# RajaeeKh/TriNerfLet

Measured on AMD Instinct MI355X. Metric: train rays/sec (whole node), higher is better.
Workload: dtype f16; 1 GPU; base: 3x32ch x 2048^2 planes, bior6.8 scale 32, hidden 64, 60000 rays/step/GPU, solid-sphere occupancy r=0.8 (re-imposed after each refresh), fp16 planes + fp16 MFMA MLP, fp32 masters, Adam+L1; GT colours = an analytic function of the ray direction (synthetic.target_colors), not a second seeded field's render; sample_budget_M=4769546, parallelism=ray-dp1

## Files before the change

include/trinerflet_hip.h:

```cpp
#ifndef TRINERFLET_HIP_H
#define TRINERFLET_HIP_H

#include <stdint.h>

#ifdef __cplusplus
extern "C" {
#endif

#define TNL_API __attribute__((visibility("default")))

TNL_API int tnl_abi_version(void);


TNL_API int tnl_near_far_from_aabb(const float *rays_o, const float *rays_d, const float *aabb,
                                   uint32_t N, float min_near, float *nears, float *fars,
                                   void *stream);

TNL_API int tnl_sph_from_ray(const float *rays_o, const float *rays_d, float radius, uint32_t N,
                             float *coords, void *stream);

TNL_API int tnl_morton3D(const int32_t *coords, uint32_t N, int32_t *indices, void *stream);

TNL_API int tnl_morton3D_invert(const int32_t *indices, uint32_t N, int32_t *coords, void *stream);

// ... 180 lines not shown
                              const float *abs_sum, float l1_coef, float *reg, void *stream);

TNL_API uint64_t tnl_permute_index(uint64_t g, uint64_t total, uint64_t key);
TNL_API int tnl_ray_batch(const float *poses, const float *intrinsics_host, uint32_t B, uint32_t H, uint32_t W,
                          const void *images, int channels, int images_u8, const int64_t *pix, uint64_t first,
                          uint64_t perm_total, uint64_t perm_key, uint32_t N, float bg_color,
                          const float *bg_rand, float *rays_o, float *rays_d, float *gt_rgb, int64_t *pix_out,
                          void *stream);

TNL_API int tnl_render_work(int units);

TNL_API int tnl_render_rays(const void *planes_tm, int half_in, uint32_t C, uint32_t R, uint32_t Hd, uint32_t Hc,
                            const void *packed, const float *rays_o, const float *rays_d, const float *nears,
                            const float *fars, uint32_t N, const uint8_t *grid, float bound, float dt_gamma,
                            uint32_t max_steps, uint32_t cascades, uint32_t H, float T_thresh, float density_scale,
                            const float *noises, int32_t *queue, float *weights_sum, float *depth, float *image,
                            void *stream);

TNL_API int tnl_infer_plan(int32_t *state, uint32_t N, uint32_t max_steps, uint32_t min_step, void *stream);
TNL_API int tnl_march_rays_dev(const int32_t *state, uint32_t N, const int32_t *rays_alive, const float *rays_t,
                               const float *rays_o, const float *rays_d, float bound, float dt_gamma,
                               uint32_t max_steps, uint32_t C, uint32_t H, const uint8_t *grid, const float *fars,
                               float *xyzs, float *dirs, float *deltas, const float *noises, float *t_scratch,
                               uint32_t rows_cap, void *stream);
TNL_API int tnl_composite_rays_dev(const int32_t *state, uint32_t N, float T_thresh, int32_t *rays_alive,
                                   float *rays_t, const float *sigmas, const float *rgbs, const float *deltas,
                                   float *weights_sum, float *depth, float *image, void *stream);
TNL_API int tnl_compact_rays_dev(int32_t *state, uint32_t N, const int32_t *rays_alive, int32_t *rays_alive_out,
                                 int32_t *workspace, void *stream);

TNL_API int tnl_idwt_level_forward_win(const float *x, const float *yh, uint32_t S, uint32_t n, int wave, float *out,
                                       const int32_t *win, void *stream);
TNL_API int tnl_idwt_level_backward_win(const float *dout, uint32_t S, uint32_t n, int wave, float *dx, float *dyh,
                                        const int32_t *win, int strided, int32_t *out_rect, void *stream);

TNL_API int tnl_idwt_set_walk_min_n(uint32_t walk_min_n);
TNL_API int tnl_idwt_get_walk_min_n(void);
TNL_API int tnl_idwt_level_forward_spans(const float *x, const float *yh, uint32_t S, uint32_t n, int wave, void *out,
                                         int half_out, const int32_t *win, int strided, const int32_t *spans,
                                         void *stream);
TNL_API int tnl_idwt_level_backward_spans(const float *dout, uint32_t S, uint32_t n, int wave, float *dx, float *dyh,
                                          const int32_t *win, int strided, int32_t *out_rect, const int32_t *spans,
                                          void *stream);
TNL_API int tnl_idwt_level_backward_live_adam(const float *dout, uint32_t S, uint32_t n, int wave, float *dx,
                                              const int32_t *win, int strided, const int32_t *live_rect,
                                              const int32_t *spans, float *p, float *m, float *v,
                                              const int32_t *band_table, uint32_t nb, const float *step_rec,
                                              float beta1, float beta2, float eps, float inv_scale,
                                              const float *inv_scale_dev, float l1_coef, const float *found_inf,
                                              float *abs_sum, void *stream);
TNL_API int tnl_planes_half_to_texel_major_spans(const void *planes_roi_half, uint32_t C, uint32_t R,
                                                 void *planes_tm_half, const int32_t *roi, const int32_t *spans,
                                                 void *stream);
TNL_API int tnl_idwt_set_tuning(int key, int value);
TNL_API int tnl_adam_l1_step_rect(float *p, float *grad, float *m, float *v, uint32_t S, uint32_t bands, uint32_t n,
                                  uint32_t spp, uint32_t s0, const int32_t *rect, float lr,
                                  const float *opt_step_dev, float beta1, float beta2, float eps, float inv_scale,
                                  const float *inv_scale_dev, float l1_coef, const float *found_inf,
                                  float *abs_sum, void *stream);
TNL_API int tnl_adam_record_step_dev(float *ring, int32_t slot, const float *lr_dev, const float *opt_step_dev, float beta1,
                                     float beta2, const float *found_inf, void *stream);
TNL_API int tnl_adam_l1_step_rec(float *p, float *grad, float *m, float *v, uint64_t n, const float *step_rec, float beta1,
                                 float beta2, float eps, const float *inv_scale_dev, float l1_coef,
                                 const float *found_inf, float *abs_sum, void *stream);
TNL_API int tnl_adam_l1_step_rect_rec(float *p, float *grad, float *m, float *v, uint32_t S, uint32_t bands, uint32_t n,
                                      uint32_t spp, uint32_t s0, const int32_t *rect, const float *step_rec, float beta1,
                                      float beta2, float eps, const float *inv_scale_dev, float l1_coef,
                                      const float *found_inf, float *abs_sum, void *stream);
TNL_API int tnl_adam_l1_step_live(float *p, float *grad, float *m, float *v, uint32_t S, uint32_t spp, uint32_t s0,
                                  uint32_t n_levels, const uint64_t *offsets, const uint32_t *sizes,
                                  const uint32_t *bands, const int32_t *live, const int32_t *grad_rect,
                                  const float *l1_coefs, float lr, const float *opt_step_dev, const float *step_rec,
                                  float beta1, float beta2, float eps, float inv_scale, const float *inv_scale_dev,
                                  const float *found_inf, float *abs_sum, void *stream);
TNL_API int tnl_adam_record_step(float *ring, int32_t slot, float lr, const float *opt_step_dev, float beta1,
                                 float beta2, const float *found_inf, void *stream);
TNL_API int tnl_adam_record_step_l1(float *ring, int32_t slot, float lr, const float *opt_step_dev, float beta1,
                                    float beta2, const float *found_inf, const float *l1_scaled_dev,
                                    const float *inv_scale_dev, void *stream);
TNL_API int tnl_adam_l1_catchup(float *p, float *m, float *v, uint32_t S, uint32_t bands, uint32_t n, uint32_t spp,
                                uint32_t s0, const int32_t *live, const float *ring, int32_t count, float beta1,
                                float beta2, float eps, float l1_coef, float *abs_sums, void *stream);
TNL_API int tnl_adam_l1_step_live_bands(float *p, float *grad, float *m, float *v, uint32_t S, uint32_t spp, uint32_t s0,
                                        uint32_t n_levels, const uint64_t *offsets, const uint32_t *sizes,
                                        const uint32_t *bands, const int32_t *live, const int32_t *grad_rect,
                                        const int32_t *const *band_tables, const uint32_t *band_quads,
                                        const float *l1_coefs, float lr, const float *opt_step_dev, const float *step_rec,
                                        float beta1, float beta2, float eps, float inv_scale, const float *inv_scale_dev,
                                        const float *found_inf, float *abs_sum, void *stream);
TNL_API int tnl_adam_l1_catchup_bands(float *p, float *m, float *v, uint32_t S, uint32_t bands, uint32_t n, uint32_t spp,
                                      uint32_t s0, const int32_t *live, const int32_t *band_table, const float *ring,
                                      int32_t count, float beta1, float beta2, float eps, float l1_coef, float *abs_sums,
                                      void *stream);

#ifdef __cplusplus
}
#endif
#endif
```

trinerflet_amd/_step/common.py:

```python
import ctypes as C_
import math
import types

import numpy as np

import torch
import torch.distributed as dist

from .. import _lib as L
from .. import distributed as D
from .. import occupancy
from .. import raymarching
from ..nerf import field as F_
from ..triplaneencoder.triplane_encoder import (_IDWTLevel, _ToTexelMajor, half_roi_into_texel_major, half_to_texel_major,
                                                idwt_level_half, idwt_level_half_roi)


def lr_factor(it, iters, warmup_steps, sched_base=0.1, warmup_factor=1e-3, sched_exp=2.5):
    w = max(warmup_steps, 0)
    if it < w:
        return sched_base * warmup_factor + it * (1 - warmup_factor) / (w - 1)
    return sched_base ** (min((it - w) / iters, 1) ** sched_exp)


class _Flat:

    def __init__(self, params):
        self.params = list(params)
        dev = self.params[0].device
        sizes = [p.numel() for p in self.params]
        self.offsets, off = [], 0
        for n in sizes:
            self.offsets.append(off)
            off += (n + 3) // 4 * 4
        self.total = off
        self.data = torch.zeros(off, dtype=torch.float32, device=dev)
        self.grad = torch.zeros(off, dtype=torch.float32, device=dev)
        self.m = torch.zeros(off, dtype=torch.float32, device=dev)
        self.v = torch.zeros(off, dtype=torch.float32, device=dev)
        for p, o, n in zip(self.params, self.offsets, sizes):
            self.data[o:o + n].copy_(p.data.reshape(-1))
            p.data = self.data[o:o + n].view(p.shape)
        self.sizes = sizes

    def grad_view(self, k):
        o, n = self.offsets[k], self.sizes[k]
        return self.grad[o:o + n].view(self.params[k].shape)

    def tune_placement(self, time_pass, candidates=12, spacing=3, good_gbs=5900.0):
        nbytes = 28.0 * self.total
        gbs = lambda ms: nbytes / (ms * 1e-3) / 1e9
        t0 = time_pass(self.data, self.grad, self.m, self.v)
        report = {"before_ms": round(t0, 4), "before_GBs": round(gbs(t0), 1), "tried_ms": []}
        best_t, best = t0, None
        hold = []
        if gbs(t0) < good_gbs:
            need = (spacing + 2) * self.data.numel() * 4
            for _ in range(candidates):
                if torch.cuda.mem_get_info(self.data.device)[0] < need:
                    report["stopped"] = "free memory"
                    break
                cand = torch.empty_like(self.data)
                hold.append(cand)
                hold.extend(torch.empty_like(self.data) for _ in range(spacing))
                t = time_pass(cand, self.grad, self.m, self.v)
                report["tried_ms"].append(round(t, 4))
                if t < best_t:
                    best_t, best = t, cand
# ... 44 lines not shown
```

trinerflet_amd/_step/planes.py:

```python
from .common import (C_, D, F_, L, _Flat, _IDWTLevel, _StepState, _ToTexelMajor, dist, half_roi_into_texel_major,
                     half_to_texel_major, idwt_level_half, idwt_level_half_roi, lr_factor, math, np, occupancy, raymarching,
                     torch, types)


class PlanesMixin:

    def _idwt_level_win(self, x, yh, win, s0=0, spans=None):
        x = x.detach().contiguous()
        yh = yh.detach().contiguous()
        P, Cc, n = x.shape[0], x.shape[1], x.shape[-1]
        out = torch.empty(P, Cc, 2 * n, 2 * n, dtype=torch.float32, device=x.device)
        L.check(L.lib().tnl_idwt_level_forward_spans(L.ptr(x), L.ptr(yh), L.u32(P * Cc), L.u32(n),
                                                     L.i32(self.enc.wave_id), L.ptr(out), L.i32(0),
                                                     L.roi_array(list(win) + [self.C, s0]), L.i32(1), L.ptr(spans),
                                                     L.stream()),
                "idwt_level_forward_spans")
        return out

    def _cropped(self, lvl):
        return self.base_res > 0 and self.crop_k > 0 and self.coef.params[lvl].shape[-1] < self.base_res

    def _crop(self, x, lvl):
        if not self._cropped(lvl):
            return x
        k = self.crop_k
        return x[..., k:-k, k:-k].contiguous()

    def rebuild_planes(self, roi=False):
        enc = self.enc
        fast = (self.J > 0 and enc.plane_dtype == torch.float16 and self.C % 8 == 0 and self.R % 16 == 0)
        if self._roi_request is not None:
            self._roi = self._finish_roi()
        roi = roi and self._roi is not None and self._tm_full is not None
        if not roi:
            self.flush_deferred()
        with torch.no_grad():
            wins = self._forward_windows() if roi else [None] * self.J
            spans, plane_spans = self._forward_spans() if roi else ([None] * self.J, None)
            if self.dist_mode == "sharded":
                planes = self._rebuild_sharded(roi, wins, spans)
            else:
                x = enc.planes_features
                for lvl in range(self.J):
                    yh = enc.planes_features_wavelet_coefs[lvl]
                    if fast and lvl == self.J - 1:
                        x = idwt_level_half_roi(x, yh, enc.wave_id, self._roi10(), spans[lvl]) if roi else \
                            idwt_level_half(x, yh, enc.wave_id)
                    elif wins[lvl] is not None:
                        x = self._idwt_level_win(x, yh, wins[lvl], spans=spans[lvl])
                    else:
                        x = _IDWTLevel.apply(x, yh, enc.wave_id)
                    x = self._crop(x, lvl)
                planes = x
            if roi:
                enc.last_used_planes = None
                enc._planes_tm = None
                enc._planes_tm_window = None
                if planes.dtype == torch.float16:
                    return half_roi_into_texel_major(planes, self._tm_full, self._roi10(), plane_spans)
                L.check(L.lib().tnl_planes_to_texel_major_win(L.ptr(planes), L.u32(self.C), L.u32(self.R), L.i32(0),
                                                              L.ptr(self._tm_full), L.roi_array(self._roi10()), L.stream()),
                        "planes_to_texel_major_win")
                return self._tm_full
            if planes.dtype == torch.float16:
                enc.last_used_planes = None
                enc._planes_tm = half_to_texel_major(planes)
            else:
                enc.last_used_planes = planes
                enc._planes_tm = _ToTexelMajor.apply(planes, enc.plane_dtype == torch.float16)
            enc._planes_tm_window = None
            self._tm_full = enc._planes_tm if self.use_roi else None
        return enc._planes_tm

    def _slice_range(self):
        return D.slice_range(3 * self.C, self.world, self.rank)

    def _rebuild_sharded(self, roi=False, wins=None, spans=None):
        enc = self.enc
        spans = spans if spans is not None else [None] * self.J
        s0, s1 = self._slice_range()
        n0 = enc.planes_features.shape[-1]
        x = enc.planes_features.reshape(3 * self.C, n0, n0)[s0:s1].unsqueeze(0).contiguous()
        fast = (self.J > 0 and enc.plane_dtype == torch.float16 and self.C % 8 == 0 and self.R % 16 == 0)
        for lvl in range(self.J):
            n = x.shape[-1]
            yh = enc.planes_features_wavelet_coefs[lvl].reshape(3 * self.C, 3, n, n)[s0:s1].unsqueeze(0).contiguous()
            if fast and lvl == self.J - 1:
                x = idwt_level_half_roi(x, yh, enc.wave_id, self._roi10(s0), spans[lvl]) if roi else \
                    idwt_level_half(x, yh, enc.wave_id)
            elif wins is not None and wins[lvl] is not None:
                x = self._idwt_level_win(x, yh, wins[lvl], s0, spans[lvl])
            else:
                x = _IDWTLevel.apply(x, yh, enc.wave_id)
            x = self._crop(x, lvl)
        if roi and x.dtype == torch.float16:
            return D.all_gather_slices(x.reshape(s1 - s0, self._roi[7], self._roi[6]), self.pg)
        if roi:
            r, C = self._roi, self.C
            xs = x.reshape(s1 - s0, self.R, self.R)
            mine = torch.empty(s1 - s0, r[7], r[6], dtype=torch.float32, device=x.device)
            for pl in range(3):
                a0, a1 = max(pl * C, s0), min((pl + 1) * C, s1)
                if a1 > a0:
                    mine[a0 - s0:a1 - s0] = xs[a0 - s0:a1 - s0, r[3 + pl]:r[3 + pl] + r[7], r[pl]:r[pl] + r[6]]
            allw = D.all_gather_slices(mine, self.pg)
            full = torch.empty(3, C, self.R, self.R, dtype=torch.float32, device=x.device)
            for pl in range(3):
                full[pl, :, r[3 + pl]:r[3 + pl] + r[7], r[pl]:r[pl] + r[6]] = allw[pl * C:(pl + 1) * C]
            return full
        mine = x.reshape(s1 - s0, self.R, self.R)
        return D.all_gather_slices(mine, self.pg).view(3, self.C, self.R, self.R)

    def _adjoint(self, grad_tm, g_cm=None, fuse=None, roi=None, scattered=False, live_adam=None):
        lib = L.lib()
        C, R = self.C, self.R
        if g_cm is None:
            g_cm = torch.empty(3, C, R, R, dtype=torch.float32, device=self.dev)
# ... 120 lines not shown
```

trinerflet_amd/csrc/wavelet.hip:

```cpp
#include <hip/hip_fp16.h>
#include <hip/hip_runtime.h>
#include <stdint.h>
#ifndef TNL_MAIN_PRIO
#define TNL_MAIN_PRIO 0
#endif
#ifndef TNL_PRIO_FWD
#define TNL_PRIO_FWD TNL_MAIN_PRIO
#endif
#ifndef TNL_PRIO_BWD
#define TNL_PRIO_BWD TNL_MAIN_PRIO
#endif
#define TNL_SET_PRIO(P) do { if (P) __builtin_amdgcn_s_setprio(P); } while (0)

#include "../../include/trinerflet_hip.h"
#include "adam_common.h"
#include "roi_common.h"

#ifndef TNL_IDWT_BWD_NT
#define TNL_IDWT_BWD_NT 1
#endif
__device__ __forceinline__ void stg(float* p, float v, bool nt) {
  if (nt) __builtin_nontemporal_store(v, p);
  else *p = v;
}
// ... 667 lines not shown
        }
        mid[0][2 * m + e][tid] = lo;
        mid[1][2 * m + e][tid] = hi;
      }
    }
    __syncthreads();
#pragma unroll
    for (int trip = 0; trip < (2 * FB * 32) / WT; trip++) {
      const int row = trip * (WT / 32) + (tid >> 5), run = tid & 31;
      const int v = 4 * run, gcol = vx0 + v;
      if (run < WV / 4 && gcol < vx1) {
        float wl[12], wh[12];
#pragma unroll
        for (int q = 0; q < 3; q++) {
          const v4f a = *reinterpret_cast<const v4f*>(&mid[0][row][v + 4 * q]);
          const v4f b = *reinterpret_cast<const v4f*>(&mid[1][row][v + 4 * q]);
#pragma unroll
          for (int i = 0; i < 4; i++) { wl[4 * q + i] = a[i]; wh[4 * q + i] = b[i]; }
        }
        float o[8];
#pragma unroll
        for (int m = 0; m < 4; m++) {
#pragma unroll
          for (int e = 0; e < 2; e++) {
            float acc = 0.f;
#pragma unroll
            for (int d = -HW; d <= HW; d++) {
              const int k = e + K - 2 * d;
              if (k >= 0 && k < L) {
                const float t0 = T.g0[k], t1 = T.g1[k];
                if (t0 != 0.f) acc = fmaf(wl[m + d + 4], t0, acc);
                if (t1 != 0.f) acc = fmaf(wh[m + d + 4], t1, acc);
              }
            }
            o[2 * m + e] = acc;
          }
        }
        const int gr = 2 * R0 + row, gc = 2 * gcol;
        const size_t off = (size_t)s * oplane + (size_t)(gr - soy) * orow + (gc - sox);
        if (HALF_OUT) {
          typedef _Float16 h8 __attribute__((ext_vector_type(8)));
          h8 hv;
#pragma unroll
          for (int i = 0; i < 8; i++) hv[i] = (_Float16)o[i];
          *reinterpret_cast<h8*>(obase + off * 2) = hv;
        } else {
          float* p = reinterpret_cast<float*>(obase) + off;
          reinterpret_cast<v4f*>(p)[0] = v4f{o[0], o[1], o[2], o[3]};
          reinterpret_cast<v4f*>(p)[1] = v4f{o[4], o[5], o[6], o[7]};
        }
      }
    }
    __syncthreads();
#pragma unroll
    for (int i = 0; i < 8; i++) { w0[i] = w0[i + FB]; w1[i] = w1[i + FB]; w2[i] = w2[i + FB]; w3[i] = w3[i + FB]; }
#pragma unroll
    for (int i = 0; i < FB; i++) { w0[8 + i] = 2.0f * n0[i]; w1[8 + i] = n1[i]; w2[8 + i] = n2[i]; w3[8 + i] = n3[i]; }
  }
}

typedef float v2f __attribute__((ext_vector_type(2)));
constexpr int PT = 64;

template <int W, bool HALF_OUT, int FB>
__global__ void __launch_bounds__(PT)
k_idwt_fwd_walk2(const float* __restrict__ x, const float* __restrict__ yh, int n, void* __restrict__ out, Roi roi,
                 int seg, LGrid lg, const int* __restrict__ spans) {
  constexpr WTaps T = wtaps(W);
  constexpr int L = T.L, K = (L - 2) / 2, HW = L / 4;
  static_assert(HW <= 4, "staged halo is 4 coarse samples");
  constexpr int WW = FB + 8;
  constexpr int LSM = WT + 4;
  __shared__ __attribute__((aligned(16))) float mid[2][2 * FB][LSM];

  int bx, by, s;
  if (!logical_block(lg, bx, by, s)) return;
  const int tid = threadIdx.x, m2 = 2 * n;
  const int pl = roi.rw ? (s + roi.s0) / roi.spp : 0;
  const int fox = roi.rw ? roi.ox[pl] : 0, foy = roi.rw ? roi.oy[pl] : 0;
  const bool compact = roi.rw && !roi.strided;
  const int orow = compact ? roi.rw : m2;
  const size_t oplane = compact ? (size_t)roi.rh * roi.rw : (size_t)m2 * m2;
  const int sox = compact ? fox : 0, soy = compact ? foy : 0;
  const int cx0 = fox / 2, cy0 = foy / 2, cw = roi.rw ? roi.rw / 2 : n, ch = roi.rw ? roi.rh / 2 : n;
  const int vx0 = cx0 + bx * WV, vx1 = min(vx0 + WV, cx0 + cw);
  int ry0 = cy0 + by * seg, ry1 = min(ry0 + seg, cy0 + ch);
  if (vx0 >= vx1 || ry0 >= ry1) return;
  __shared__ int s_span[2];
  if (spans != nullptr && !narrow_rows(spans, n, pl, vx0, vx1, ry0, ry1, s_span)) return;
  const int c = vx0 - 4 + 2 * tid;
  const bool col_ok = c >= 0 && c < n && c < vx1 + 4;
  const size_t nn = (size_t)n * n;
  const float* b0 = x + (size_t)s * nn + (col_ok ? c : 0);
  const float* b1 = yh + (size_t)s * 3 * nn + (col_ok ? c : 0);
  auto ld4 = [&](int r, v2f& v0, v2f& v1, v2f& v2, v2f& v3) {
    v0 = v1 = v2 = v3 = v2f{0.f, 0.f};
    if (col_ok && r >= 0 && r < n) {
      const size_t o = (size_t)r * n;
      v0 = *reinterpret_cast<const v2f*>(b0 + o); v1 = *reinterpret_cast<const v2f*>(b1 + o);
      v2 = *reinterpret_cast<const v2f*>(b1 + nn + o); v3 = *reinterpret_cast<const v2f*>(b1 + 2 * nn + o);
    }
  };
  v2f w0[WW], w1[WW], w2[WW], w3[WW];
  v2f n0[FB], n1[FB], n2[FB], n3[FB];
#pragma unroll
  for (int i = 0; i < WW; i++) ld4(ry0 - 4 + i, w0[i], w1[i], w2[i], w3[i]);
// ... 480 lines not shown
}

inline int pick_tpw(uint32_t ntx, uint32_t nty, uint32_t S) {
  int tpw = TPW_MAX;
  while (tpw > 1 && (uint64_t)cdiv(ntx, tpw) * nty * S < 3000) tpw >>= 1;
  return tpw;
}
inline int pick_seg(uint32_t tiles, uint32_t rows, uint32_t S) {
  int seg = 256;
  while (seg > 32 && (uint64_t)tiles * cdiv(rows, seg) * S < 12000) seg >>= 1;
  return seg;
}

template <int W>
int launch_fwd(const float* x, const float* yh, uint32_t S, uint32_t n, void* out, int half_out, hipStream_t st,
               Roi roi = Roi{}, const int* spans = nullptr) {
  if (spans != nullptr && !(roi.rw && n % 8 == 0 && (int)n >= g_walk_min_n)) spans = nullptr;
  if (n % 8 == 0 && (int)n >= g_walk_min_n) {
    const uint32_t cw = roi.rw ? roi.rw / 2 : n, ch = roi.rw ? roi.rh / 2 : n;
    const uint32_t tiles = cdiv(cw, WV);
    const int seg = g_seg ? g_seg : pick_seg(tiles, ch, S);
    dim3 grid;
    LGrid lg;
    walk_grid(tiles, cdiv(ch, seg), S, grid, lg);
#define TNL_FWD_WALK(HALF, FB) \
  hipLaunchKernelGGL((k_idwt_fwd_walk<W, HALF, FB>), grid, dim3(WT), 0, st, x, yh, (int)n, out, roi, seg, lg, spans)
#define TNL_FWD_WALK2(HALF, FB) \
  hipLaunchKernelGGL((k_idwt_fwd_walk2<W, HALF, FB>), grid, dim3(PT), 0, st, x, yh, (int)n, out, roi, seg, lg, spans)
    bool pair = g_fwd_pair != 0 && cw % 2 == 0;
    if (roi.rw) for (int p = 0; p < 3; p++) pair = pair && roi.ox[p] % 4 == 0;
    if (pair) {
      if (half_out) { if (g_fwd_pair == 2) TNL_FWD_WALK2(true, 2); else TNL_FWD_WALK2(true, 4); }
      else { if (g_fwd_pair == 2) TNL_FWD_WALK2(false, 2); else TNL_FWD_WALK2(false, 4); }
    } else if (half_out) { if (g_fwd_fb == 4) TNL_FWD_WALK(true, 4); else TNL_FWD_WALK(true, 8); }
    else { if (g_fwd_fb == 4) TNL_FWD_WALK(false, 4); else TNL_FWD_WALK(false, 8); }
#undef TNL_FWD_WALK
#undef TNL_FWD_WALK2
  } else if (n % 4 == 0) {
    const uint32_t ntx = roi.rw ? roi.rw / (2 * TI) : cdiv(n, TI), nty = roi.rw ? roi.rh / (2 * TI) : cdiv(n, TI);
    const int tpw = pick_tpw(ntx, nty, S);
    const dim3 grid(cdiv(ntx, tpw), nty, S);
    if (half_out)
      hipLaunchKernelGGL((k_idwt_fwd_pipe<W, true>), grid, dim3(NT), 0, st, x, yh, (int)n, out, roi, tpw);
    else
      hipLaunchKernelGGL((k_idwt_fwd_pipe<W, false>), grid, dim3(NT), 0, st, x, yh, (int)n, out, roi, tpw);
  } else {
    if (roi.rw) return (int)hipErrorInvalidValue;
    if (half_out) return (int)hipErrorInvalidValue;
    hipLaunchKernelGGL(k_idwt_fwd<W>, dim3(cdiv(n, TI), cdiv(n, TI), S), dim3(NT), 0, st, x, yh, (int)n,
                       reinterpret_cast<float*>(out));
  }
  return (int)hipGetLastError();
}
template <int W>
int launch_bwd(const float* dout, uint32_t S, uint32_t n, float* dx, float* dyh, hipStream_t st, Roi roi = Roi{},
               int32_t* out_rect = nullptr, const int* spans = nullptr) {
  Roi orect{};
  if (out_rect != nullptr) {
    const bool walk = n % 8 == 0 && (int)n >= g_walk_min_n;
    const int G = walk ? 8 : TI;
    if (n % 2 != 0 || n % G != 0) return (int)hipErrorInvalidValue;
    constexpr WTaps T = wtaps(W);
    constexpr int L = T.L, K = (L - 2) / 2, KA = (K + 3) / 4 * 4, SH = KA - K;
    const int FT = 2 * G + L - 2, FTA = (2 * G + L - 2 + SH + 3) / 4 * 4;
    const int nt = (int)n / G;
    int lo[2][3], hi[2][3];
    for (int p = 0; p < 3; p++) {
      const int wo[2] = {roi.rw ? roi.ox[p] : 0, roi.rw ? roi.oy[p] : 0};
      const int we[2] = {roi.rw ? roi.rw : 2 * (int)n, roi.rw ? roi.rh : 2 * (int)n};
      const int ka[2] = {KA, K}, ft[2] = {FTA, FT};
      for (int d = 0; d < 2; d++) {
        lo[d][p] = nt; hi[d][p] = -1;
        for (int t = 0; t < nt; t++) {
          const int c0 = 2 * t * G - ka[d];
          if (c0 < wo[d] + we[d] && c0 + ft[d] > wo[d]) { lo[d][p] = t < lo[d][p] ? t : lo[d][p]; hi[d][p] = t; }
        }
        if (hi[d][p] < 0) { lo[d][p] = 0; hi[d][p] = 0; }
      }
    }
    int ext[2] = {0, 0};
    for (int d = 0; d < 2; d++)
      for (int p = 0; p < 3; p++) ext[d] = (hi[d][p] - lo[d][p] + 1) > ext[d] ? (hi[d][p] - lo[d][p] + 1) : ext[d];
    for (int p = 0; p < 3; p++) {
      orect.ox[p] = G * (lo[0][p] + ext[0] > nt ? nt - ext[0] : lo[0][p]);
      orect.oy[p] = G * (lo[1][p] + ext[1] > nt ? nt - ext[1] : lo[1][p]);
      out_rect[p] = orect.ox[p]; out_rect[3 + p] = orect.oy[p];
    }
    orect.rw = G * ext[0]; orect.rh = G * ext[1];
    out_rect[6] = orect.rw; out_rect[7] = orect.rh;
    orect.spp = roi.rw ? roi.spp : (int)(S / 3);
    orect.s0 = roi.s0;
  }
  if (n % 8 == 0 && (int)n >= g_walk_min_n) {
    const uint32_t ow = orect.rw ? orect.rw : n, oh = orect.rw ? orect.rh : n;
    const uint32_t tiles = cdiv(ow, AVC);
    const int seg = g_seg ? g_seg : pick_seg(tiles, oh, S);
    dim3 grid;
    LGrid lg;
    walk_grid(tiles, cdiv(oh, seg), S, grid, lg);
    if (spans != nullptr && (out_rect == nullptr || dx == nullptr)) return (int)hipErrorInvalidValue;
    hipLaunchKernelGGL((k_idwt_bwd_walk<W, false>), grid, dim3(AT), 0, st, dout, (int)n, dx, dyh, roi, orect, seg, lg, spans,
                       WalkAdam{});
  } else if (n % 2 == 0) {
    const int tpw = pick_tpw(cdiv(n, TI), cdiv(n, TI), S);
    hipLaunchKernelGGL((k_idwt_bwd_pipe<W, false>), dim3(cdiv(cdiv(n, TI), tpw), cdiv(n, TI), S), dim3(NT), 0, st, dout,
                       (int)n, dx, dyh, FuseAdam{}, roi, orect, tpw);
// ... 60 lines not shown
    case 1: return launch_fwd<1>(x, yh, S, n, out, half_out, st, roi, spans);
    case 2: return launch_fwd<2>(x, yh, S, n, out, half_out, st, roi, spans);
    case 3: return launch_fwd<3>(x, yh, S, n, out, half_out, st, roi, spans);
    case 4: return launch_fwd<4>(x, yh, S, n, out, half_out, st, roi, spans);
    default: return (int)hipErrorInvalidValue;
  }
}

int tnl_idwt_level_forward(const float* x, const float* yh, uint32_t S, uint32_t n, int wave, float* out,
                           void* stream) {
  return idwt_forward_any(x, yh, S, n, wave, out, 0, stream);
}

int tnl_idwt_level_forward_half(const float* x, const float* yh, uint32_t S, uint32_t n, int wave, void* out_half,
                                void* stream) {
  if (n % 4 != 0) return (int)hipErrorInvalidValue;
  return idwt_forward_any(x, yh, S, n, wave, out_half, 1, stream);
}

int tnl_idwt_level_forward_half_roi(const float* x, const float* yh, uint32_t S, uint32_t n, int wave, void* out_half,
                                    const int32_t* roi, void* stream) {
  if (n % 4 != 0) return (int)hipErrorInvalidValue;
  return idwt_forward_any(x, yh, S, n, wave, out_half, 1, stream, roi);
}

int tnl_idwt_level_forward_win(const float* x, const float* yh, uint32_t S, uint32_t n, int wave, float* out,
                               const int32_t* win, void* stream) {
  if (n % 4 != 0) return (int)hipErrorInvalidValue;
  return idwt_forward_any(x, yh, S, n, wave, out, 0, stream, win, 1);
}

static int planes_half_to_tm(const void* planes_cm_half, uint32_t C, uint32_t R, void* planes_tm_half,
                             const int32_t* roi_host, void* stream, const int32_t* spans = nullptr);

int tnl_idwt_level_forward_spans(const float* x, const float* yh, uint32_t S, uint32_t n, int wave, void* out,
                                 int half_out, const int32_t* win, int strided, const int32_t* spans, void* stream) {
  if (n % 4 != 0 || win == nullptr) return (int)hipErrorInvalidValue;
  return idwt_forward_any(x, yh, S, n, wave, out, half_out, stream, win, strided, spans);
}

int tnl_planes_half_to_texel_major_spans(const void* planes_roi_half, uint32_t C, uint32_t R, void* planes_tm_half,
                                         const int32_t* roi, const int32_t* spans, void* stream) {
  return planes_half_to_tm(planes_roi_half, C, R, planes_tm_half, roi, stream, spans);
}

int tnl_planes_half_to_texel_major_roi(const void* planes_roi_half, uint32_t C, uint32_t R, void* planes_tm_half,
                                       const int32_t* roi, void* stream) {
  return planes_half_to_tm(planes_roi_half, C, R, planes_tm_half, roi, stream);
}

int tnl_planes_half_to_texel_major(const void* planes_cm_half, uint32_t C, uint32_t R, void* planes_tm_half,
                                   void* stream) {
  return planes_half_to_tm(planes_cm_half, C, R, planes_tm_half, nullptr, stream);
}

static int planes_half_to_tm(const void* planes_cm_half, uint32_t C, uint32_t R, void* planes_tm_half,
                             const int32_t* roi_host, void* stream, const int32_t* spans) {
  if (C == 0 || R == 0) return 0;
  if (C % 8 != 0 || R % 8 != 0) return (int)hipErrorInvalidValue;
  Roi roi;
  if (!make_roi(roi_host, 3 * C, R, roi) || (roi.rw && (roi.spp != (int)C || roi.s0 != 0)))
    return (int)hipErrorInvalidValue;
  constexpr int TY = TNL_LAYOUT_ROWS;
  static_assert(TY == 1 || TY == 2 || TY == 4 || TY == 8, "rows per workgroup must divide the spans' 8-row groups");
  const uint32_t rows = roi.rw ? (uint32_t)roi.rh : R;
  const dim3 grid = roi.rw ? dim3(roi.rw / TX, cdiv(rows, TY), 3) : dim3(cdiv(R, TX), cdiv(rows, TY), 3);
  const size_t lds = (size_t)TY * ((size_t)C * (TX + 8) + (C / 8) * 8) * sizeof(_Float16);
  hipLaunchKernelGGL(k_to_texel_major_h<TY>, grid, dim3(NT), lds, (hipStream_t)stream,
                     reinterpret_cast<const _Float16*>(planes_cm_half), (int)C, (int)R,
                     reinterpret_cast<_Float16*>(planes_tm_half), roi, roi.rw ? spans : nullptr);
  return (int)hipGetLastError();
}

static int idwt_backward_any(const float* dout, uint32_t S, uint32_t n, int wave, float* dx, float* dyh,
                             const int32_t* roi_host, void* stream, int strided = 0, int32_t* out_rect = nullptr,
                             const int32_t* spans = nullptr);

int tnl_idwt_level_backward_spans(const float* dout, uint32_t S, uint32_t n, int wave, float* dx, float* dyh,
                                  const int32_t* win, int strided, int32_t* out_rect, const int32_t* spans,
                                  void* stream) {
  if (win == nullptr) return (int)hipErrorInvalidValue;
  if (!(n % 8 == 0 && (int)n >= g_walk_min_n)) spans = nullptr;
  return idwt_backward_any(dout, S, n, wave, dx, dyh, win, stream, strided, out_rect, spans);
}

int tnl_idwt_level_backward(const float* dout, uint32_t S, uint32_t n, int wave, float* dx, float* dyh,
                            void* stream) {
  return idwt_backward_any(dout, S, n, wave, dx, dyh, nullptr, stream);
}

int tnl_idwt_level_backward_roi(const float* dout_roi, uint32_t S, uint32_t n, int wave, float* dx, float* dyh,
                                const int32_t* roi, void* stream) {
  return idwt_backward_any(dout_roi, S, n, wave, dx, dyh, roi, stream);
}

int tnl_idwt_level_backward_win(const float* dout, uint32_t S, uint32_t n, int wave, float* dx, float* dyh,
                                const int32_t* win, int strided, int32_t* out_rect, void* stream) {
  return idwt_backward_any(dout, S, n, wave, dx, dyh, win, stream, strided, out_rect);
}

static int idwt_backward_any(const float* dout, uint32_t S, uint32_t n, int wave, float* dx, float* dyh,
                             const int32_t* roi_host, void* stream, int strided, int32_t* out_rect,
                             const int32_t* spans) {
  if (S == 0 || n == 0) return 0;
  if (S > 65535) return (int)hipErrorInvalidValue;
  Roi roi;
// ... 113 lines not shown
```

trinerflet_amd/triplaneencoder/triplane_encoder.py:

```python
import weakref

import torch
import torch.nn as nn
import torch.nn.functional as F
from torch.autograd import Function

from .. import _lib as L
from . import utils

WAVELET_IDS = {'haar': 0, 'bior2.2': 1, 'bior4.4': 2, 'bior2.6': 3, 'bior6.8': 4}
PAD_DICT = {'bior6.8': 4, 'bior2.6': 3, 'bior4.4': 2, 'bior2.2': 1, 'haar': 0}
_REC = {
    'haar': ([0.7071067811865476, 0.7071067811865476], [0.7071067811865476, -0.7071067811865476]),
    'bior2.2': ([0, 0.3535533905932738, 0.7071067811865476, 0.3535533905932738, 0, 0],
                [0, 0.1767766952966369, 0.3535533905932738, -1.0606601717798212, 0.3535533905932738,
                 0.1767766952966369]),
    'bior4.4': ([0, -0.06453888262869706, -0.04068941760916406, 0.41809227322161724, 0.7884856164055829,
                 0.41809227322161724, -0.04068941760916406, -0.06453888262869706, 0, 0],
                [0, -0.03782845550726404, -0.023849465019556843, 0.11062440441843718, 0.37740285561283066,
                 -0.8526986790088938, 0.37740285561283066, 0.11062440441843718, -0.023849465019556843,
                 -0.03782845550726404]),
    'bior2.6': ([0, 0, 0, 0, 0, 0.3535533905932738, 0.7071067811865476, 0.3535533905932738, 0, 0, 0, 0, 0, 0],
                [0, 0.006905339660024878, 0.013810679320049757, -0.04695630968816917, -0.1077232986963881,
                 0.16987135563661201, 0.4474660099696121, -0.966747552403483, 0.4474660099696121,
# ... 81 lines not shown
            dyh = torch.zeros(3, C, 3, n, n, dtype=torch.float32, device=dev)
            rect = (ctypes.c_int32 * 8)()
            L.check(lib.tnl_idwt_level_backward_win(L.ptr(g), L.u32(3 * C), L.u32(n), L.i32(wave_id), L.ptr(dx), L.ptr(dyh),
                                                    L.roi_array(win + [C, 0]), L.i32(1), rect, L.stream()),
                    "idwt_level_backward_win")
            win = list(rect)
            grads[lvl] = dyh
            rects[lvl] = list(rect)
            g = dx
        from .. import occupancy
        live = occupancy.live_rects(ctx.fwd_wins, rects, [R >> (J - lvl) for lvl in range(J)])
        for lvl, ref in enumerate(ctx.coef_refs):
            prm = ref()
            if prm is not None:
                prm._tnl_live = (live[lvl], rects[lvl], roi, grads[lvl].data_ptr(), grads[lvl]._version)
        return (None, None, g, *grads)


def idwt_level_half(x, yh, wave_id):
    x = x.detach().to(torch.float32).contiguous()
    yh = yh.detach().to(torch.float32).contiguous()
    P, C, n = x.shape[0], x.shape[1], x.shape[-1]
    out = torch.empty(P, C, 2 * n, 2 * n, dtype=torch.float16, device=x.device)
    L.check(L.lib().tnl_idwt_level_forward_half(L.ptr(x), L.ptr(yh), L.u32(P * C), L.u32(n), L.i32(wave_id),
                                                L.ptr(out), L.stream()), "idwt_level_forward_half")
    return out


def idwt_level_half_roi(x, yh, wave_id, roi, spans=None):
    x = x.detach().to(torch.float32).contiguous()
    yh = yh.detach().to(torch.float32).contiguous()
    P, C, n = x.shape[0], x.shape[1], x.shape[-1]
    out = torch.empty(P * C, roi[7], roi[6], dtype=torch.float16, device=x.device)
    L.check(L.lib().tnl_idwt_level_forward_spans(L.ptr(x), L.ptr(yh), L.u32(P * C), L.u32(n), L.i32(wave_id),
                                                 L.ptr(out), L.i32(1), L.roi_array(roi), L.i32(0), L.ptr(spans),
                                                 L.stream()),
            "idwt_level_forward_spans")
    return out


def half_roi_into_texel_major(planes_roi_half, tm, roi, spans=None):
    _, R, _, C = tm.shape
    L.check(L.lib().tnl_planes_half_to_texel_major_spans(L.ptr(planes_roi_half), L.u32(C), L.u32(R), L.ptr(tm),
                                                         L.roi_array(roi), L.ptr(spans), L.stream()),
            "planes_half_to_texel_major_spans")
    return tm


def half_to_texel_major(planes_cm_half):
    _, C, R, _ = planes_cm_half.shape
    tm = torch.empty(3, R, R, C, dtype=torch.float16, device=planes_cm_half.device)
    L.check(L.lib().tnl_planes_half_to_texel_major(L.ptr(planes_cm_half), L.u32(C), L.u32(R), L.ptr(tm), L.stream()),
            "planes_half_to_texel_major")
    return tm


class _ToTexelMajor(Function):

    @staticmethod
    def forward(ctx, planes_cm, half, window=None):
        L.require_cuda(planes_cm)
        planes_cm = planes_cm.to(torch.float32).contiguous()
        _, C, R, _ = planes_cm.shape
        tm = torch.empty(3, R, R, C, dtype=torch.float16 if half else torch.float32, device=planes_cm.device)
        if window is not None:
            L.check(L.lib().tnl_planes_to_texel_major_win(L.ptr(planes_cm), L.u32(C), L.u32(R), L.i32(1 if half else 0),
                                                          L.ptr(tm), L.roi_array(list(window) + [C, 0]), L.stream()),
                    "planes_to_texel_major_win")
            return tm
        L.check(L.lib().tnl_planes_to_texel_major(L.ptr(planes_cm), L.u32(C), L.u32(R), L.i32(1 if half else 0),
                                                  L.ptr(tm), L.stream()), "planes_to_texel_major")
        return tm

    @staticmethod
    def backward(ctx, g_tm):
        g_tm = g_tm.to(torch.float32).contiguous()
        _, R, _, C = g_tm.shape
        g_cm = torch.empty(3, C, R, R, dtype=torch.float32, device=g_tm.device)
        L.check(L.lib().tnl_planes_to_channel_major(L.ptr(g_tm), L.u32(C), L.u32(R), L.ptr(g_cm), L.stream()),
                "planes_to_channel_major")
        return g_cm, None, None


class _Sample(Function):

    @staticmethod
    def forward(ctx, planes_tm, xyz, bound):
        L.require_cuda(planes_tm, xyz)
        xyz = xyz.to(torch.float32).contiguous()
        _, R, _, C = planes_tm.shape
        N = xyz.shape[0]
        feats = torch.empty(N, 3 * C, dtype=torch.float32, device=xyz.device)
        L.check(L.lib().tnl_triplane_sample_forward(L.ptr(planes_tm), L.i32(int(planes_tm.dtype == torch.float16)),
                                                    L.ptr(xyz), L.f32(bound), L.u32(N), L.u32(C), L.u32(R),
                                                    L.ptr(feats), L.stream()), "triplane_sample_forward")
        ctx.save_for_backward(xyz)
        ctx.dims = (C, R, float(bound))
        return feats

    @staticmethod
    def backward(ctx, g):
        (xyz,) = ctx.saved_tensors
        C, R, bound = ctx.dims
        g = g.to(torch.float32).contiguous()
        g_tm = torch.zeros(3, R, R, C, dtype=torch.float32, device=g.device)
        L.check(L.lib().tnl_triplane_sample_backward(L.ptr(g), L.ptr(xyz), L.f32(bound), L.u32(xyz.shape[0]),
# ... 510 lines not shown
```

Measured before the change: 9.634 million rays/s.

## Fuse final IDWT level with texel-major fp16 transpose into one kernel

Adds a walk kernel that computes the last inverse wavelet level and writes its fp16 output straight into the texel-major [3,R,R,C] plane array. Each block stages channel groups through LDS, so one texel's channels are stored as a single 16-byte vector. This removes the separate channel-major half-precision plane buffer and the extra transpose kernel that read it back. In exchange it uses more shared memory and a wider thread block. It also scatters stores per texel, which could lower occupancy or store efficiency.

Result: no change. 9.615 million rays/s (-0.2%).

```diff
diff --git a/include/trinerflet_hip.h b/include/trinerflet_hip.h
--- a/include/trinerflet_hip.h
+++ b/include/trinerflet_hip.h
@@ -256,6 +256,12 @@
 TNL_API int tnl_planes_half_to_texel_major_spans(const void *planes_roi_half, uint32_t C, uint32_t R,
                                                  void *planes_tm_half, const int32_t *roi, const int32_t *spans,
                                                  void *stream);
+TNL_API int tnl_idwt_level_forward_texel_major_supported(uint32_t C, uint32_t n, int wave);
+TNL_API int tnl_idwt_level_forward_texel_major(const float *x, const float *yh, uint32_t C, uint32_t n, int wave,
+                                               void *planes_tm_half, void *stream);
+TNL_API int tnl_idwt_level_forward_texel_major_spans(const float *x, const float *yh, uint32_t C, uint32_t n, int wave,
+                                                     void *planes_tm_half, const int32_t *roi, const int32_t *spans,
+                                                     const int32_t *plane_spans, void *stream);
 TNL_API int tnl_idwt_set_tuning(int key, int value);
 TNL_API int tnl_adam_l1_step_rect(float *p, float *grad, float *m, float *v, uint32_t S, uint32_t bands, uint32_t n,
                                   uint32_t spp, uint32_t s0, const int32_t *rect, float lr,
diff --git a/trinerflet_amd/_step/common.py b/trinerflet_amd/_step/common.py
--- a/trinerflet_amd/_step/common.py
+++ b/trinerflet_amd/_step/common.py
@@ -13,7 +13,8 @@
 from .. import raymarching
 from ..nerf import field as F_
 from ..triplaneencoder.triplane_encoder import (_IDWTLevel, _ToTexelMajor, half_roi_into_texel_major, half_to_texel_major,
-                                                idwt_level_half, idwt_level_half_roi)
+                                                idwt_level_half, idwt_level_half_roi, idwt_level_texel_major,
+                                                idwt_texel_major_supported)
 
 
 def lr_factor(it, iters, warmup_steps, sched_base=0.1, warmup_factor=1e-3, sched_exp=2.5):
diff --git a/trinerflet_amd/_step/planes.py b/trinerflet_amd/_step/planes.py
--- a/trinerflet_amd/_step/planes.py
+++ b/trinerflet_amd/_step/planes.py
@@ -1,6 +1,6 @@
 from .common import (C_, D, F_, L, _Flat, _IDWTLevel, _StepState, _ToTexelMajor, dist, half_roi_into_texel_major,
-                     half_to_texel_major, idwt_level_half, idwt_level_half_roi, lr_factor, math, np, occupancy, raymarching,
-                     torch, types)
+                     half_to_texel_major, idwt_level_half, idwt_level_half_roi, idwt_level_texel_major,
+                     idwt_texel_major_supported, lr_factor, math, np, occupancy, raymarching, torch, types)
 
 
 class PlanesMixin:
@@ -37,12 +37,20 @@
         with torch.no_grad():
             wins = self._forward_windows() if roi else [None] * self.J
             spans, plane_spans = self._forward_spans() if roi else ([None] * self.J, None)
+            direct = (fast and self.dist_mode != "sharded" and not self._cropped(self.J - 1) and
+                      idwt_texel_major_supported(self.C, enc.planes_features_wavelet_coefs[-1].shape[-1], enc.wave_id))
+            tm = None
             if self.dist_mode == "sharded":
                 planes = self._rebuild_sharded(roi, wins, spans)
             else:
                 x = enc.planes_features
                 for lvl in range(self.J):
                     yh = enc.planes_features_wavelet_coefs[lvl]
+                    if direct and lvl == self.J - 1:
+                        tm = idwt_level_texel_major(x, yh, enc.wave_id, self._tm_full, self._roi10(), spans[lvl],
+                                                    plane_spans) if roi else idwt_level_texel_major(x, yh, enc.wave_id)
+                        x = None
+                        break
                     if fast and lvl == self.J - 1:
                         x = idwt_level_half_roi(x, yh, enc.wave_id, self._roi10(), spans[lvl]) if roi else \
                             idwt_level_half(x, yh, enc.wave_id)
@@ -56,13 +64,18 @@
                 enc.last_used_planes = None
                 enc._planes_tm = None
                 enc._planes_tm_window = None
+                if tm is not None:
+                    return tm
                 if planes.dtype == torch.float16:
                     return half_roi_into_texel_major(planes, self._tm_full, self._roi10(), plane_spans)
                 L.check(L.lib().tnl_planes_to_texel_major_win(L.ptr(planes), L.u32(self.C), L.u32(self.R), L.i32(0),
                                                               L.ptr(self._tm_full), L.roi_array(self._roi10()), L.stream()),
                         "planes_to_texel_major_win")
                 return self._tm_full
-            if planes.dtype == torch.float16:
+            if tm is not None:
+                enc.last_used_planes = None
+                enc._planes_tm = tm
+            elif planes.dtype == torch.float16:
                 enc.last_used_planes = None
                 enc._planes_tm = half_to_texel_major(planes)
             else:
diff --git a/trinerflet_amd/csrc/wavelet.hip b/trinerflet_amd/csrc/wavelet.hip
--- a/trinerflet_amd/csrc/wavelet.hip
+++ b/trinerflet_amd/csrc/wavelet.hip
@@ -743,6 +743,141 @@
       }
     }
     __syncthreads();
+#pragma unroll
+    for (int i = 0; i < 8; i++) { w0[i] = w0[i + FB]; w1[i] = w1[i + FB]; w2[i] = w2[i + FB]; w3[i] = w3[i + FB]; }
+#pragma unroll
+    for (int i = 0; i < FB; i++) { w0[8 + i] = 2.0f * n0[i]; w1[8 + i] = n1[i]; w2[8 + i] = n2[i]; w3[8 + i] = n3[i]; }
+  }
+}
+
+template <int W, int FB, int G>
+__global__ void __launch_bounds__(WT * G)
+k_idwt_fwd_walk_tm(const float* __restrict__ x, const float* __restrict__ yh, int n, int C, _Float16* __restrict__ tm,
+                   Roi roi, int seg, LGrid lg, const int* __restrict__ spans, const int* __restrict__ pspans) {
+  TNL_SET_PRIO(TNL_PRIO_FWD);
+  constexpr WTaps T = wtaps(W);
+  constexpr int L = T.L, K = (L - 2) / 2, HW = L / 4;
+  static_assert(HW <= 4, "staged halo is 4 coarse samples");
+  static_assert(G == 4 || G == 8, "a texel's channel group is one 8- or 16-byte store");
+  constexpr int WW = FB + 8;
+  constexpr int LSM = WT + 4;
+  constexpr int SLD = 2 * WV + 8;
+  typedef _Float16 h8 __attribute__((ext_vector_type(8)));
+  typedef _Float16 hG __attribute__((ext_vector_type(G)));
+  __shared__ __attribute__((aligned(16))) float mid_all[G][2][2 * FB][LSM];
+  __shared__ __attribute__((aligned(16))) _Float16 stage[2 * FB][G][SLD];
+
+  int bxg, by, pl;
+  if (!logical_block(lg, bxg, by, pl)) return;
+  const int ncg = C / G;
+  const int cg = bxg % ncg, bx = bxg / ncg;
+  const int tid = threadIdx.x, ty = threadIdx.y, m2 = 2 * n;
+  const int s = pl * C + cg * G + ty;
+  float (*mid)[2 * FB][LSM] = mid_all[ty];
+  const int fox = roi.rw ? roi.ox[pl] : 0, foy = roi.rw ? roi.oy[pl] : 0;
+  const int cx0 = fox / 2, cy0 = foy / 2, cw = roi.rw ? roi.rw / 2 : n, ch = roi.rw ? roi.rh / 2 : n;
+  const int vx0 = cx0 + bx * WV, vx1 = min(vx0 + WV, cx0 + cw);
+  int ry0 = cy0 + by * seg, ry1 = min(ry0 + seg, cy0 + ch);
+  if (vx0 >= vx1 || ry0 >= ry1) return;
+  __shared__ int s_span[2];
+  if (spans != nullptr && !narrow_rows(spans, n, pl, vx0, vx1, ry0, ry1, s_span)) return;
+  const int c = vx0 - 4 + tid;
+  const bool col_ok = c >= 0 && c < n && c < vx1 + 4;
+  const size_t nn = (size_t)n * n;
+  const float* b0 = x + (size_t)s * nn + (col_ok ? c : 0);
+  const float* b1 = yh + (size_t)s * 3 * nn + (col_ok ? c : 0);
+  auto ld4 = [&](int r, float& v0, float& v1, float& v2, float& v3) {
+    v0 = v1 = v2 = v3 = 0.f;
+    if (col_ok && r >= 0 && r < n) {
+      const size_t o = (size_t)r * n;
+      v0 = b0[o]; v1 = b1[o]; v2 = b1[nn + o]; v3 = b1[2 * nn + o];
+    }
+  };
+  float w0[WW], w1[WW], w2[WW], w3[WW];
+  float n0[FB], n1[FB], n2[FB], n3[FB];
+#pragma unroll
+  for (int i = 0; i < WW; i++) ld4(ry0 - 4 + i, w0[i], w1[i], w2[i], w3[i]);
+#pragma unroll
+  for (int i = 0; i < WW; i++) w0[i] *= 2.0f;
+  const int fw = 2 * (vx1 - vx0);
+  const int lin = ty * WT + tid;
+  _Float16* const tbase = tm + ((size_t)pl * m2 * m2 + 2 * vx0) * C + cg * G;
+  for (int R0 = ry0; R0 < ry1; R0 += FB) {
+    const bool more = R0 + FB < ry1;
+    if (more) {
+#pragma unroll
+      for (int i = 0; i < FB; i++) ld4(R0 + FB + 4 + i, n0[i], n1[i], n2[i], n3[i]);
+    }
+#pragma unroll
+    for (int m = 0; m < FB; m++) {
+#pragma unroll
+      for (int e = 0; e < 2; e++) {
+        float lo = 0.f, hi = 0.f;
+#pragma unroll
+        for (int d = -HW; d <= HW; d++) {
+          const int k = e + K - 2 * d;
+          if (k >= 0 && k < L) {
+            const float t0 = T.g0[k], t1 = T.g1[k];
+            if (t0 != 0.f) { lo = fmaf(w0[m + d + 4], t0, lo); hi = fmaf(w2[m + d + 4], t0, hi); }
+            if (t1 != 0.f) { lo = fmaf(w1[m + d + 4], t1, lo); hi = fmaf(w3[m + d + 4], t1, hi); }
+          }
+        }
+        mid[0][2 * m + e][tid] = lo;
+        mid[1][2 * m + e][tid] = hi;
+      }
+    }
+    __syncthreads();
+#pragma unroll
+    for (int trip = 0; trip < (2 * FB * 32) / WT; trip++) {
+      const int row = trip * (WT / 32) + (tid >> 5), run = tid & 31;
+      const int v = 4 * run, gcol = vx0 + v;
+      if (run < WV / 4 && gcol < vx1) {
+        float wl[12], wh[12];
+#pragma unroll
+        for (int q = 0; q < 3; q++) {
+          const v4f a = *reinterpret_cast<const v4f*>(&mid[0][row][v + 4 * q]);
+          const v4f b = *reinterpret_cast<const v4f*>(&mid[1][row][v + 4 * q]);
+#pragma unroll
+          for (int i = 0; i < 4; i++) { wl[4 * q + i] = a[i]; wh[4 * q + i] = b[i]; }
+        }
+        h8 hv;
+#pragma unroll
+        for (int m = 0; m < 4; m++) {
+#pragma unroll
+          for (int e = 0; e < 2; e++) {
+            float acc = 0.f;
+#pragma unroll
+            for (int d = -HW; d <= HW; d++) {
+              const int k = e + K - 2 * d;
+              if (k >= 0 && k < L) {
+                const float t0 = T.g0[k], t1 = T.g1[k];
+                if (t0 != 0.f) acc = fmaf(wl[m + d + 4], t0, acc);
+                if (t1 != 0.f) acc = fmaf(wh[m + d + 4], t1, acc);
+              }
+            }
+            hv[2 * m + e] = (_Float16)acc;
+          }
+        }
+        *reinterpret_cast<h8*>(&stage[row][ty][2 * v]) = hv;
+      }
+    }
+    __syncthreads();
+    for (int idx = lin; idx < 2 * FB * 2 * WV; idx += WT * G) {
+      const int row = idx / (2 * WV), col = idx - row * (2 * WV);
+      const int y = 2 * R0 + row, xg = 2 * vx0 + col;
+      bool ok = col < fw;
+      if (ok && pspans != nullptr) {
+        const int* ps = pspans + ((size_t)pl * (m2 >> 3) + (y >> 3)) * 2;
+        const int p0 = fox + ((xg - fox) & ~(TX - 1));
+        ok = ps[0] < p0 + TX && ps[1] > p0;
+      }
+      if (ok) {
+        hG o;
+#pragma unroll
+        for (int j = 0; j < G; j++) o[j] = stage[row][j][col];
+        *reinterpret_cast<hG*>(tbase + ((size_t)y * m2 + col) * C) = o;
+      }
+    }
 #pragma unroll
     for (int i = 0; i < 8; i++) { w0[i] = w0[i + FB]; w1[i] = w1[i + FB]; w2[i] = w2[i + FB]; w3[i] = w3[i + FB]; }
 #pragma unroll
@@ -1329,6 +1464,24 @@
   }
   return (int)hipGetLastError();
 }
+constexpr int TMG = 8;
+inline bool fwd_tm_ok(uint32_t C, uint32_t n, int wave) {
+  return wave >= 1 && wave <= 4 && C != 0 && C % TMG == 0 && n % 8 == 0 && (int)n >= g_walk_min_n && 3ull * C <= 65535;
+}
+template <int W>
+int launch_fwd_tm(const float* x, const float* yh, uint32_t C, uint32_t n, _Float16* tm, hipStream_t st, Roi roi,
+                  const int* spans, const int* pspans) {
+  const uint32_t cw = roi.rw ? roi.rw / 2 : n, ch = roi.rw ? roi.rh / 2 : n;
+  const uint32_t tiles = cdiv(cw, WV);
+  const int seg = g_seg ? g_seg : pick_seg(tiles, ch, 3 * C);
+  dim3 grid;
+  LGrid lg;
+  walk_grid(tiles * (C / TMG), cdiv(ch, seg), 3, grid, lg);
+  hipLaunchKernelGGL((k_idwt_fwd_walk_tm<W, 4, TMG>), grid, dim3(WT, TMG), 0, st, x, yh, (int)n, (int)C, tm, roi, seg, lg,
+                     roi.rw ? spans : nullptr, roi.rw ? pspans : nullptr);
+  return (int)hipGetLastError();
+}
+
 template <int W>
 int launch_bwd(const float* dout, uint32_t S, uint32_t n, float* dx, float* dyh, hipStream_t st, Roi roi = Roi{},
                int32_t* out_rect = nullptr, const int* spans = nullptr) {
@@ -1495,6 +1648,31 @@
 int tnl_planes_half_to_texel_major(const void* planes_cm_half, uint32_t C, uint32_t R, void* planes_tm_half,
                                    void* stream) {
   return planes_half_to_tm(planes_cm_half, C, R, planes_tm_half, nullptr, stream);
+}
+
+int tnl_idwt_level_forward_texel_major_supported(uint32_t C, uint32_t n, int wave) { return fwd_tm_ok(C, n, wave) ? 1 : 0; }
+
+int tnl_idwt_level_forward_texel_major_spans(const float* x, const float* yh, uint32_t C, uint32_t n, int wave,
+                                             void* planes_tm_half, const int32_t* roi_host, const int32_t* spans,
+                                             const int32_t* plane_spans, void* stream) {
+  if (!fwd_tm_ok(C, n, wave)) return (int)hipErrorInvalidValue;
+  Roi roi;
+  if (!make_roi(roi_host, 3 * C, 2 * n, roi) || (roi.rw && (roi.spp != (int)C || roi.s0 != 0)))
+    return (int)hipErrorInvalidValue;
+  hipStream_t st = (hipStream_t)stream;
+  _Float16* tm = reinterpret_cast<_Float16*>(planes_tm_half);
+  switch (wave) {
+    case 1: return launch_fwd_tm<1>(x, yh, C, n, tm, st, roi, spans, plane_spans);
+    case 2: return launch_fwd_tm<2>(x, yh, C, n, tm, st, roi, spans, plane_spans);
+    case 3: return launch_fwd_tm<3>(x, yh, C, n, tm, st, roi, spans, plane_spans);
+    case 4: return launch_fwd_tm<4>(x, yh, C, n, tm, st, roi, spans, plane_spans);
+    default: return (int)hipErrorInvalidValue;
+  }
+}
+
+int tnl_idwt_level_forward_texel_major(const float* x, const float* yh, uint32_t C, uint32_t n, int wave,
+                                       void* planes_tm_half, void* stream) {
+  return tnl_idwt_level_forward_texel_major_spans(x, yh, C, n, wave, planes_tm_half, nullptr, nullptr, nullptr, stream);
 }
 
 static int planes_half_to_tm(const void* planes_cm_half, uint32_t C, uint32_t R, void* planes_tm_half,
diff --git a/trinerflet_amd/triplaneencoder/triplane_encoder.py b/trinerflet_amd/triplaneencoder/triplane_encoder.py
--- a/trinerflet_amd/triplaneencoder/triplane_encoder.py
+++ b/trinerflet_amd/triplaneencoder/triplane_encoder.py
@@ -157,6 +157,27 @@
     tm = torch.empty(3, R, R, C, dtype=torch.float16, device=planes_cm_half.device)
     L.check(L.lib().tnl_planes_half_to_texel_major(L.ptr(planes_cm_half), L.u32(C), L.u32(R), L.ptr(tm), L.stream()),
             "planes_half_to_texel_major")
+    return tm
+
+
+def idwt_texel_major_supported(C, n, wave_id):
+    return bool(L.lib().tnl_idwt_level_forward_texel_major_supported(L.u32(C), L.u32(n), L.i32(wave_id)))
+
+
+def idwt_level_texel_major(x, yh, wave_id, tm=None, roi=None, spans=None, plane_spans=None):
+    x = x.detach().to(torch.float32).contiguous()
+    yh = yh.detach().to(torch.float32).contiguous()
+    _, C, n = x.shape[0], x.shape[1], x.shape[-1]
+    if tm is None:
+        if roi is not None:
+            raise ValueError("a windowed rebuild needs the array it updates")
+        tm = torch.empty(3, 2 * n, 2 * n, C, dtype=torch.float16, device=x.device)
+    if tuple(tm.shape) != (3, 2 * n, 2 * n, C) or tm.dtype != torch.float16 or not tm.is_contiguous():
+        raise ValueError("tm must be a contiguous fp16 [3,2n,2n,C] array")
+    L.check(L.lib().tnl_idwt_level_forward_texel_major_spans(L.ptr(x), L.ptr(yh), L.u32(C), L.u32(n), L.i32(wave_id),
+                                                             L.ptr(tm), L.roi_array(roi), L.ptr(spans),
+                                                             L.ptr(plane_spans), L.stream()),
+            "idwt_level_forward_texel_major_spans")
     return tm
 
 
```
